# chlhnu/DOT-SOCP

Hardware: AMD Instinct MI355X
Metric: ADMM iters/sec on NxNxT dot2d staggered grid at 1/2/4/8 MI355X (higher is better)
Workload: dtype f64

## Files before the change

### dot-socp_amd/capi.py

```python
import ctypes
import os

import numpy as np

_HERE = os.path.dirname(os.path.abspath(__file__))
LIB_PATH = os.path.join(_HERE, "lib", "libdotsocp.so")

i64 = ctypes.c_longlong
dbl = ctypes.c_double
vp = ctypes.c_void_p


class DotsocpError(RuntimeError):
    def __init__(self, code, msg):
        super().__init__(f"libdotsocp error {code}: {msg}")
        self.code = code


class Problem(ctypes.Structure):
    _fields_ = [("dim", ctypes.c_int), ("weighted", ctypes.c_int),
                ("ny", i64), ("nx", i64), ("nt", i64),
                ("D", dbl), ("E", dbl), ("cScale", dbl), ("dScale", dbl),
                ("normc", dbl), ("normd", dbl)]

# ... 15 lines not shown


METHOD_INPALM, METHOD_PALM, METHOD_ACCADMM = 0, 1, 2


F_PHI, F_Q, F_ALPHA, F_Z, F_BETA, F_C, F_WEIGHT = range(7)

SYMBOLS = {
    "dotsocp_last_error": (ctypes.c_char_p, []),
    "dotsocp_version": (ctypes.c_char_p, []),
    "dotsocp_device_count": (ctypes.c_int, []),
    "dotsocp_proj_soc": (ctypes.c_int, [vp, vp, i64, i64]),
    "dotsocp_bfd": (ctypes.c_int, [vp, vp, i64, i64, i64, dbl, dbl]),
    "dotsocp_bfd_conj": (ctypes.c_int, [vp, vp, i64, i64, i64, dbl]),
    "dotsocp_bfd1d": (ctypes.c_int, [vp, vp, i64, i64, dbl, dbl]),
    "dotsocp_bfd_conj1d": (ctypes.c_int, [vp, vp, i64, i64, dbl]),
    "dotsocp_oper_poisson": (ctypes.c_int, [vp, vp, i64, i64, i64, dbl]),
    "dotsocp_dctn": (ctypes.c_int, [vp, i64, i64, i64, ctypes.c_int]),
    "dotsocp_proj_soc_dev": (ctypes.c_int, [vp, vp, i64, i64, vp]),
    "dotsocp_bfd_dev": (ctypes.c_int, [vp, vp, i64, i64, i64, dbl, dbl, vp]),
    "dotsocp_bfd_conj_dev": (ctypes.c_int, [vp, vp, i64, i64, i64, dbl, vp]),
    "dotsocp_create": (vp, [ctypes.POINTER(Problem), ctypes.c_int, ctypes.c_int]),
    "dotsocp_create_multi": (vp, [ctypes.POINTER(Problem), ctypes.c_int, ctypes.c_int]),
    "dotsocp_destroy": (None, [vp]),
    "dotsocp_rccl_unique_id": (ctypes.c_int, [vp]),
    "dotsocp_attach_rccl": (ctypes.c_int, [vp, vp, ctypes.c_int, ctypes.c_int]),
    "dotsocp_slab_range": (ctypes.c_int, [i64, ctypes.c_int, ctypes.c_int, ctypes.POINTER(i64), ctypes.POINTER(i64)]),
    "dotsocp_field_len": (i64, [ctypes.POINTER(Problem), ctypes.c_int]),
    "dotsocp_dct_algorithm": (ctypes.c_int, [i64]),
    "dotsocp_tsolve_tri_safe": (ctypes.c_int, [i64, i64, i64]),
    "dotsocp_cone_writes_beta": (ctypes.c_int, [i64, dbl, i64, ctypes.c_int, ctypes.c_int, ctypes.c_int, dbl, dbl]),
    "dotsocp_rescale_due": (ctypes.c_int, [i64, ctypes.c_int, dbl, dbl]),
    "dotsocp_qcone_form": (ctypes.c_int, [i64, dbl, i64, ctypes.c_int, ctypes.c_int, ctypes.c_int, ctypes.c_int, dbl, dbl]),
    "dotsocp_release_cache": (i64, []),
    "dotsocp_upload": (ctypes.c_int, [vp, ctypes.c_int, vp]),
    "dotsocp_upload_layers": (ctypes.c_int, [vp, ctypes.c_int, vp, i64, i64]),
    "dotsocp_download": (ctypes.c_int, [vp, ctypes.c_int, vp]),
    "dotsocp_begin": (ctypes.c_int, [vp, ctypes.POINTER(Opts)]),
    "dotsocp_begin_method": (ctypes.c_int, [vp, ctypes.POINTER(Opts), ctypes.c_int, ctypes.POINTER(AccOpts)]),
    "dotsocp_run": (ctypes.c_int, [vp, i64, ctypes.POINTER(i64)]),
    "dotsocp_recover_outputs": (ctypes.c_int, [vp, vp, vp, vp, vp, vp, vp, vp, vp]),
    "dotsocp_jump_next_level": (ctypes.c_int, [vp, vp]),
    "dotsocp_finish": (ctypes.c_int, [vp, ctypes.POINTER(Result)]),
    "dotsocp_get_history": (ctypes.c_int, [vp, vp, vp, vp, vp]),
    "dotsocp_set_profiling": (ctypes.c_int, [vp, ctypes.c_int]),
    "dotsocp_kernel_time": (ctypes.c_int, [vp, ctypes.c_char_p, ctypes.POINTER(dbl), ctypes.POINTER(i64)]),
    "dotsocp_canary_check": (ctypes.c_int, []),
    "dotsocp_poisson_phi": (ctypes.c_int, [vp]),
    "dotsocp_synchronize": (ctypes.c_int, [vp]),
}

_lib = None


def _share_torchs_hip_runtime():
    import importlib.util
    import sys
    if "torch" in sys.modules or os.environ.get("DOTSOCP_SYSTEM_HIP"):
        return
    try:
        spec = importlib.util.find_spec("torch")
    except (ImportError, ValueError):
        return
    if not spec or not spec.submodule_search_locations:
        return
    for name in ("libamdhip64.so", "libamdhip64.so.7"):
# ... 55 lines not shown
```

### dot-socp_amd/csrc/capi.hip

```cpp
#include <cstring>
#include <new>

#include "comm.h"
#include "solver.h"

using namespace dotsocp;

namespace dotsocp {
extern thread_local std::string g_last_error;
int dotsocp_slab_range_impl(i64 nt, int world, int rank, i64 *t0, i64 *t1);
}

struct dotsocp_ctx {
    Solver s;
};

static int require_device() {
    int n = 0;
    if (hipGetDeviceCount(&n) != hipSuccess || n <= 0) {
        set_error("no HIP device available (libdotsocp has no CPU fallback)");
        return DOTSOCP_ENODEVICE;
    }
    return 0;
}
// ... 234 lines not shown
    ncclUniqueId uid;
    static_assert(sizeof(uid) == 128, "ncclUniqueId is expected to be 128 bytes");
    DS_NCCL(api.GetUniqueId(&uid));
    memcpy(id, &uid, sizeof uid);
    return 0;
}

int dotsocp_attach_rccl(dotsocp_ctx *ctx, const unsigned char id[128], int rank, int world) {
    if (!ctx) { set_error("ctx is NULL"); return DOTSOCP_EINVAL; }
    return ctx->s.attach_rccl(id, rank, world);
}

#define CTX_OR_FAIL()                                      \
    do {                                                   \
        if (!ctx) { set_error("ctx is NULL"); return DOTSOCP_EINVAL; } \
        (void)hipGetLastError();    \
    } while (0)

int dotsocp_dct_algorithm(dotsocp_i64 n) { return dct_choose_algorithm(n); }
int dotsocp_tsolve_tri_safe(dotsocp_i64 ny, dotsocp_i64 nx, dotsocp_i64 nt) { return tsolve_tri_safe(ny, nx, nt) ? 1 : 0; }

int dotsocp_cone_writes_beta(dotsocp_i64 it, double last_sigma_it, dotsocp_i64 maxit, int check_step_by_step,
                             int last_of_run, int rescale, double maxFeas, double relGap) {
    return cone_writes_beta(it, last_sigma_it, maxit, check_step_by_step != 0, last_of_run != 0, rescale, maxFeas, relGap) ? 1 : 0;
}
int dotsocp_rescale_due(dotsocp_i64 it, int rescale, double maxFeas, double relGap) {
    return rescale_due(it, rescale, maxFeas, relGap) ? 1 : 0;
}
int dotsocp_qcone_form(dotsocp_i64 it, double last_sigma_it, dotsocp_i64 maxit, int check_step_by_step, int last_of_run,
                       int next_last_of_run, int rescale, double maxFeas, double relGap) {
    return qcone_form(it, last_sigma_it, maxit, check_step_by_step != 0, last_of_run != 0, next_last_of_run != 0, rescale,
                      maxFeas, relGap);
}

dotsocp_i64 dotsocp_field_len(const dotsocp_problem *p, int field) {
    if (!p || (p->dim != 1 && p->dim != 2) || p->nt < 2 || p->nx < 1 || (p->dim == 2 && p->ny < 1)) return -1;
    const i64 ny = p->dim == 1 ? p->nx : p->ny, nx = p->dim == 1 ? 1 : p->nx, nt = p->nt;
    const i64 Nphi = ny * nx * nt, Nz = ny * nx * (nt - 1);
    const i64 Nq = Nz + ny * (nx - 1) * nt + (ny - 1) * nx * nt;
    switch (field) {
        case DOTSOCP_F_PHI: case DOTSOCP_F_C: return Nphi;
        case DOTSOCP_F_Q: case DOTSOCP_F_ALPHA: case DOTSOCP_F_WEIGHT: return Nq;
        case DOTSOCP_F_Z: case DOTSOCP_F_BETA: return Nz * (p->dim == 1 ? 6 : 10);
        default: return -1;
    }
}

int dotsocp_upload(dotsocp_ctx *ctx, int field, const double *host) { CTX_OR_FAIL(); return ctx->s.upload(field, host); }
dotsocp_i64 dotsocp_release_cache(void) { return (dotsocp_i64)device_cache_release(); }

int dotsocp_upload_layers(dotsocp_ctx *ctx, int field, const double *host, dotsocp_i64 t0, dotsocp_i64 n) {
    CTX_OR_FAIL();
    return ctx->s.upload_layers(field, host, t0, n);
}
int dotsocp_download(dotsocp_ctx *ctx, int field, double *host) { CTX_OR_FAIL(); return ctx->s.download(field, host); }
int dotsocp_begin(dotsocp_ctx *ctx, const dotsocp_opts *opts) { CTX_OR_FAIL(); return ctx->s.begin(opts); }
int dotsocp_begin_method(dotsocp_ctx *ctx, const dotsocp_opts *opts, int method, const dotsocp_acc_opts *acc) {
    CTX_OR_FAIL();
    return ctx->s.begin_method(opts, method, acc);
}
int dotsocp_recover_outputs(dotsocp_ctx *ctx, const double *rho0, const double *rho1, double *rho, double *Ex,
                            double *Ey, double *q0, double *bx, double *by) {
    CTX_OR_FAIL();
    if (ctx->s.prob.dim == 1)
        return ctx->s.recover_outputs(rho0, rho1, rho, nullptr, Ex, q0, nullptr, bx);
    return ctx->s.recover_outputs(rho0, rho1, rho, Ex, Ey, q0, bx, by);
// ... 63 lines not shown
```

### dot-socp_amd/csrc/kernels.h

```cpp
#pragma once
#include "common.h"
#include "defer.h"

namespace dotsocp {

struct LoopCoef {
    double s;
    double sf;
    double dF;
    double at, ax, ay;
    double tau;
    double c1, c2;
    double dinv1, dinv2;
};

enum {
    S_Q2 = 0, S_Z2, S_APHI2, S_ALPHA2, S_BETA2, S_FBBETA2, S_PRIM1, S_PRIM2, S_DUAL1, S_DUAL2,
    S_COMPLEM, S_DOTCOMP, S_RHO2, S_RHOFQ2, S_MRHOB, S_M2, S_RHOB2, S_QALPHA, S_CPHI, S_PHI2,
    S_COUNT
};

struct KktCoef {
    double sigma;
    double kappa;
// ... 88 lines not shown
                        double sc_in1, double sc_out, hipStream_t st, i64 tc0 = 0, i64 Nzc = -1);
int launch_scale_div(double *x, const double *w, i64 n, double sc, hipStream_t st);
int launch_fill(double *x, i64 n, double v, hipStream_t st);
int launch_outputs(const Grid &g, const double *q, const double *alpha, const double *weight, const double *rho0,
                   const double *rho1, const double *a_prev, double sig, double cD, double dD, int which, double *out,
                   hipStream_t st);
int launch_out_tail(const Grid &g, const double *alpha, const double *weight, double sig, double cD, double *out,
                    hipStream_t st);

int launch_qstep_fused(const Grid &g, const LoopCoef &c, const FusedGeom &fg, const double *phi,
                       const double *q2, const double *sx, const double *sy, const double *weight,
                       const double *tail_bx, const double *tail_by, double *q_out, double *alpha,
                       hipStream_t st);
struct QStepExtra {
    ScaleOps aops;
    double *partials, *resid;
    double kappa, dsD;
    double *u0_tail;
    int c_ends;
};
int launch_qstep_rhs(const Grid &g, const LoopCoef &c, const FusedGeom &fg, const double *phi, const double *q2,
                     const double *sx, const double *sy, const double *weight, const double *tail_bx,
                     const double *tail_by, const double *cvec, double *q_out, const double *alpha_in, double *alpha_out,
                     double *rhs, hipStream_t st, i64 z0 = 0, i64 zcount = -1, i64 zstride = 1,
                     const QStepExtra *ex = nullptr);
i64 qstep_rhs_blocks(const Grid &g, const FusedGeom &fg);
struct QConeArgs {
    const double *phi, *q2v, *sx, *sy, *cvec, *alpha_in, *gamma_in;
    double *alpha_out, *rhs, *q_out, *beta_out, *q2_out, *sx_out, *sy_out;
    i64 TC;
    int ap_on;
    double ap_mul, ap_div;
    int c_ends;
};
int launch_qcone(const Grid &g, const LoopCoef &c, const FusedGeom &fg, QConeArgs a, bool gout, hipStream_t st);
i64 qcone_chunk_len(const Grid &g);
int launch_rhs_sigma_fix(const Grid &g, double *rhs, const double *r, double *cvec, double factor, hipStream_t st,
                         bool c_ends = false);
int launch_c_interior_test(const Grid &g, const double *cvec, int *flag, hipStream_t st);
i64 qstep_rhs_chunks(const Grid &g, const FusedGeom &fg, i64 *TC = nullptr);
int launch_qstep_rhs_acc(int var, const Grid &g, const LoopCoef &c, const FusedGeom &fg, const double *phi,
                         const double *q2, const double *sx, const double *sy, const double *weight, const double *cvec,
                         double *q_raw, const double *alpha_in, double *alpha_out, double *rhs, double *q_state,
                         const double *q_anchor, const double *alpha_anchor, const AccCoef &k, hipStream_t st,
                         const double *tail_bx = nullptr, const double *tail_by = nullptr, double *u0_tail = nullptr);
int launch_rhs_fixup(const Grid &g, const LoopCoef &c, const double *u0_prev, double *rhs, hipStream_t st);
int launch_qstep_palm_first(const Grid &g, const LoopCoef &c, const FusedGeom &fg, const double *phi, const double *q2,
                            const double *sx, const double *sy, const double *cvec, double *q_out, const double *alpha,
                            double *rhs, hipStream_t st, const double *tail_bx = nullptr, const double *tail_by = nullptr,
                            const double *qk = nullptr);
int launch_grad(const Grid &g, const LoopCoef &c, const double *phi, double *out, hipStream_t st);
int launch_tail_finalize(const Grid &g, const LoopCoef &c, const FusedGeom &fg, const double *q2, const double *sx,
                         const double *sy, double *tail_bx, double *tail_by, hipStream_t st);
int launch_kkt_tail(const Grid &g, const double *alpha, const double *beta, const double *weight, double *a0,
                    double *a0w, double *bt_bx, double *bt_by, hipStream_t st);
int launch_rhs(const Grid &g, const LoopCoef &c, const double *q, const double *alpha, const double *cvec,
               const double *weight, const double *u0_prev, double *rhs, hipStream_t st, bool c_ends = false);
int launch_qstep(const Grid &g, const LoopCoef &c, const double *phi, const double *z, const double *beta,
                 const double *weight, const double *tail_bx, const double *tail_by, double *q,
                 double *alpha, hipStream_t st);
int launch_u0_tail(const Grid &g, const double *q, const double *alpha, const double *weight, double *out,
                   hipStream_t st);
int launch_scale(double *x, i64 n, double mul, double div, hipStream_t st);
#define DS_MAX_WORLD 64
struct PencilCuts {
    int world;
    i64 cut[DS_MAX_WORLD + 1];
};
// ... 71 lines not shown
```

### dot-socp_amd/csrc/solver.h

```cpp
#pragma once
#include <chrono>
#include <functional>
#include <memory>
#include <string>
#include <vector>

#include "hostmem.h"
#include "kernels.h"

namespace dotsocp {

int guarded_malloc(void **p, size_t bytes);
void guarded_free(void *p);
long long device_cache_release();
int canary_check(std::string *report);
bool canary_enabled();
bool stream_stress_enabled();
void stream_stress(hipStream_t st);

template <class T>
inline int dmalloc(T **p, i64 n) {
    *p = nullptr;
    if (n <= 0) n = 1;
    return guarded_malloc((void **)p, sizeof(T) * (size_t)n);
// ... 44 lines not shown
    i64 l0 = 0, nl = 0;
    double *pencil = nullptr, *pencil2 = nullptr;
    double *stage = nullptr;
    double *u0_prev = nullptr, *tail_bx = nullptr, *tail_by = nullptr;
    double *a0_prev = nullptr, *a0w_prev = nullptr, *btail_bx = nullptr, *btail_by = nullptr;
    double *send_plane = nullptr, *send_plane2 = nullptr, *send_bx = nullptr, *send_by = nullptr;
    KktWork kw{};
    double *q_old = nullptr, *q2 = nullptr, *beta2 = nullptr, *sx = nullptr, *sy = nullptr;
    double *q3 = nullptr, *p2 = nullptr, *sxp = nullptr, *syp = nullptr;
    double *send_pbx = nullptr, *send_pby = nullptr, *ptail_bx = nullptr, *ptail_by = nullptr;
    double *alpha2 = nullptr;
    double *sx2 = nullptr, *sy2 = nullptr;
    double *tri_send = nullptr, *tri_recv = nullptr, *tri_bsend = nullptr, *tri_brecv = nullptr, *tri_zero = nullptr;
    double *carry = nullptr;
    FusedGeom fg{};
    double *phi_p = nullptr, *alpha_p = nullptr, *z_p = nullptr;
    double *phi_a = nullptr, *q_a = nullptr, *alpha_a = nullptr, *z_a = nullptr, *beta_a = nullptr;
};

#define FOR_SLABS(s) for (auto &s : slabs) if (int rc_use__ = use(s)) return rc_use__; else

int dotsocp_slab_range_impl(i64 nt, int world, int rank, i64 *t0, i64 *t1);
void pencil_range(i64 plane, int world, int j, i64 *l0, i64 *l1);

bool if_adjust_sigma(double iter, double last_iter);

enum Phase { PH_RHS = 0, PH_POISSON, PH_PROJ, PH_QSTEP, PH_BETA, PH_KKT, PH_FUSED_A, PH_FUSED_B, PH_MATERIALISE,
             PH_COMM, PH_INTERP, PH_ACC_CONE, PH_ACC_GATHER, PH_QSTEP0, PH_TRANSPOSE, PH_CONE_CARRY, PH_QCONE, PH_COUNT };

bool rescale_due(i64 it, int rescale, double maxFeas, double relGap);
bool cone_writes_beta(i64 it, double lastSigmaIt, i64 maxit, bool checkStepByStep, bool last_of_run, int rescale,
                      double maxFeas, double relGap);

enum { QCONE_NONE = 0, QCONE_STEADY = 1, QCONE_EXIT = 2 };
int qcone_form(i64 it, double lastSigmaIt, i64 maxit, bool checkStepByStep, bool last_of_run, bool next_last_of_run,
               int rescale, double maxFeas, double relGap);

struct Solver {
    dotsocp_problem prob{};
    int device = 0;
    i64 ny = 0, nx = 0, nt = 0;
    hipStream_t stream = nullptr;
    hipStream_t stream_z = nullptr;
    bool multi_device = false;
    int ndev_visible = 1;
    std::vector<DevRes *> devres;
    int cur_dev = -1;
    std::vector<Slab> slabs;
    std::unique_ptr<DeferCtx> defer;
    int world = 1;
    int rank = 0;
    void *nccl = nullptr;
    double *h_sums = nullptr;
    double *d_red = nullptr;
    bool fused = true;
    bool overlap = false;
    bool tri_tsolve = true;
    bool peer_ok = true;
    bool cross_device = false;
    ~Solver();
    int init(const dotsocp_problem *p, int device, int nslabs, bool multi_dev = false);
    int attach_rccl(const unsigned char *id, int rank, int world);
    int use(const Slab &s);
    int use_dev(int d);
    int sync_all();
    DevRes *res_for(int dev);
    i64 column_pad() const;
    i64 row_pitch() const;
    int alloc_slabs(int first, int count);
// ... 164 lines not shown
```

### dot-socp_amd/csrc/solver.hip

```cpp
#include "solver.h"

#include <algorithm>
#include <cmath>
#include <cstring>

#include "comm.h"

namespace dotsocp {

void Solver::update_coef() {
    lc.s = E / D;
    lc.sf = edge_factor(lc.s);
    lc.dF = E / dScale;
    const double ht = 1.0 / (double)(nt - 1);
    lc.at = D * (1.0 / ht);
    lc.ax = (nx > 1) ? D * (1.0 / (1.0 / (double)(nx - 1))) : 0.0;
    lc.ay = (ny > 1) ? D * (1.0 / (1.0 / (double)(ny - 1))) : 0.0;
    lc.tau = opts.tau;
    const double tmp = (E / D) * (E / D);
    if (prob.weighted) { lc.c1 = 2.0 * tmp; lc.c2 = tmp; }
    else { lc.c1 = 1.0 + 2.0 * tmp; lc.c2 = 1.0 + tmp; }
    lc.dinv1 = 1.0 / lc.c1;
    lc.dinv2 = 1.0 / lc.c2;
}
// ... 302 lines not shown
        }
        const int mode = deferred ? 1 : 0;
        if (s.carry && C > 1) {
            for (i64 z = z0; z < z0 + zc; ++z) {
                a.carry_in = (z > 0) ? s.carry : nullptr;
                a.carry_out = (z + 1 < C) ? s.carry : nullptr;
                DS_CHECK(launch_cone_fused(mode, s.g, lc, s.fg, a, s.st, z, 1, flavour));
            }
        } else {
            DS_CHECK(launch_cone_fused(mode, s.g, lc, s.fg, a, s.st, z0, zc, flavour));
        }
        if (deferred && part != 1) std::swap(s.beta, s.beta2);
    }
    prof_end(ph);
    if (part == 1) return 0;
    if (deferred) {
        bops.clear();
        beta_gamma = gout;
    }
    return 0;
}

KktCoef Solver::kkt_coef() const {
    KktCoef k;
    k.sigma = sigma;
    k.kappa = sigma * cScale * D;
    k.dsD = dScale / D;
    k.dsE = dScale / E;
    return k;
}

int Solver::phase_q(int part, bool kkt, int early) {
    if (!fused) DS_CHECK(flush_alpha());
    if (early != QCONE_NONE && (part != 0 || kkt || multi() || !fused || !deferred || !beta_gamma || !bops.empty())) {
        set_error("internal: early cone pass in a state it does not serve");
        return DOTSOCP_ESTATE;
    }
    const bool egout = (early == QCONE_STEADY);
    const int ph = (early != QCONE_NONE) ? PH_QCONE : PH_QSTEP;
    prof_begin(ph);
    FOR_SLABS(s) {
        hipStream_t st = s.st;
        if (early != QCONE_NONE && qcone != 2) {
            if (!s.sx2) {
                DS_CHECK(s.zalloc(&s.sx2, s.fg.sx_len));
                DS_CHECK(s.zalloc(&s.sy2, s.fg.sy_len));
            }
            QConeArgs a{};
            a.phi = s.phi; a.q2v = s.q2; a.sx = s.sx; a.sy = s.sy; a.cvec = s.c; a.alpha_in = s.alpha; a.gamma_in = s.beta;
            a.alpha_out = s.alpha2; a.rhs = s.w0; a.q_out = s.q_old; a.beta_out = s.beta2;
            a.q2_out = s.q; a.sx_out = s.sx2; a.sy_out = s.sy2;
            a.ap_on = aops.n; a.ap_mul = aops.mul; a.ap_div = aops.div;
            a.c_ends = (c_ends_on && s.c_ends) ? 1 : 0;
            DS_CHECK(launch_qcone(s.g, lc, s.fg, a, egout, st));
            std::swap(s.alpha, s.alpha2);
            std::swap(s.q, s.q_old);
            std::swap(s.q2, s.q_old);
            std::swap(s.sx, s.sx2);
            std::swap(s.sy, s.sy2);
            std::swap(s.beta, s.beta2);
        } else if (!fused) {
            DS_CHECK(launch_qstep(s.g, lc, s.phi, s.z, s.beta, s.weight, s.tail_bx, s.tail_by, s.q, s.alpha, s.st));
        } else {
            const i64 C = qstep_rhs_chunks(s.g, s.fg);
            i64 z0 = 0, zc = C, zs = 1;
            if (part == 1) { zc = C - 1; }
            else if (part == 2) { z0 = C - 1; zc = 1; }
            QStepExtra ex{};
            ex.aops = aops;
            ex.c_ends = (c_ends_on && s.c_ends) ? 1 : 0;
            if (multi() && !s.g.last && part != 1) ex.u0_tail = s.send_plane;
            if (kkt) {
                const KktCoef k = kkt_coef();
                ex.partials = kkt_qstep_partials(s.g, s.kw);
                ex.resid = s.w1;
                ex.kappa = k.kappa; ex.dsD = k.dsD;
            }
            DS_CHECK(launch_qstep_rhs(s.g, lc, s.fg, s.phi, s.q2, s.sx, s.sy, s.weight, s.tail_bx, s.tail_by, s.c,
                                      s.q_old, s.alpha, s.alpha2, s.w0, st, z0, zc, zs, &ex));
            if (part != 1) std::swap(s.alpha, s.alpha2);
            if (part != 1) std::swap(s.q, s.q_old);
            if (early != QCONE_NONE) {
                FusedArgs a{};
                a.q = s.q; a.q2 = s.q2; a.sx = s.sx; a.sy = s.sy;
                a.beta_in = s.beta; a.beta_out = s.beta2;
                a.bops = bops;
                DS_CHECK(launch_cone_fused(1, s.g, lc, s.fg, a, s.st, 0, s.fg.chunks, CONE_GIN | (egout ? CONE_GOUT : 0)));
                std::swap(s.beta, s.beta2);
            }
        }
    }
    prof_end(ph);
    if (part == 1) return 0;
    q_valid = true;
    if (early != QCONE_NONE) {
        q_valid = !egout || qcone == 2;
        beta_gamma = egout;
        z_valid = false;
        z_prev_ok = false;
        early_pass = true;
        early_gout = egout;
    }
    u0_made = multi() && fused;
    if (fused) aops.clear();
    rhs_valid = fused;
    if (multi() && fused && comm_z && cone_split_enabled()) halo_pending = true;
    else DS_CHECK(exchange_q_halo(true));
    return 0;
}

int Solver::phase_mult() {
    if (fused) {
        deferred = true;
        return 0;
    }
    prof_begin(PH_BETA);
    FOR_SLABS(s) DS_CHECK(launch_beta_update(s.g, lc, s.q, s.z, s.beta, s.st));
    prof_end(PH_BETA);
    return 0;
}

int Solver::materialise() {
    if (!fused || !deferred) return 0;
    DS_CHECK(need_beta_form("materialise"));
    DS_CHECK(need_q("materialise"));
    DS_CHECK(ensure_halo());
    prof_begin(PH_MATERIALISE);
    FOR_SLABS(s) {
        FusedArgs a = pending_step_args(s);
        a.beta_out = s.beta;
// ... 180 lines not shown
    dScale = dScale2 * dScale;
    cScale = cScale2 * cScale;
    sigmaScale = sigmaScale * (cScale2 / dScale2);
    update_coef();
    rescale += 1;
    return 0;
}

bool rescale_due(i64 it, int rescale, double maxFeas, double relGap) {
    if (rescale >= 3 && (it % 100) == 0) return true;
    if (rescale == 1 && maxFeas < 2e-2 && it >= 10 && relGap < 5e-2) return true;
    if (rescale == 2 && maxFeas < 5e-3 && it >= 50 && relGap < 1e-2) return true;
    return false;
}

bool cone_writes_beta(i64 it, double lastSigmaIt, i64 maxit, bool checkStepByStep, bool last_of_run, int rescale,
                      double maxFeas, double relGap) {
    if (checkStepByStep || if_adjust_sigma((double)it, lastSigmaIt) || it >= maxit) return true;
    if (last_of_run) return true;
    return rescale_due(it + 1, rescale, maxFeas, relGap);
}

int qcone_form(i64 it, double lastSigmaIt, i64 maxit, bool checkStepByStep, bool last_of_run, bool next_last_of_run,
               int rescale, double maxFeas, double relGap) {
    if (cone_writes_beta(it, lastSigmaIt, maxit, checkStepByStep, last_of_run, rescale, maxFeas, relGap)) return QCONE_NONE;
    return cone_writes_beta(it + 1, lastSigmaIt, maxit, checkStepByStep, next_last_of_run, rescale, maxFeas, relGap)
               ? QCONE_EXIT : QCONE_STEADY;
}

bool Solver::time_limit_passed() const {
    return timeout_pending || (remote() ? false : (elapsed() > time_limit || (timeout_at > 0 && it >= timeout_at)));
}

int Solver::qcone_decide() const {
    if (qcone == 0 || !fused || multi() || prob.weighted || method != DOTSOCP_METHOD_INPALM) return QCONE_NONE;
    if (!deferred || !beta_gamma || !bops.empty()) return QCONE_NONE;
    const Slab &s = slabs[0];
    if (s.g.ncl < 1 || s.fg.XB != 4) return QCONE_NONE;
    if (qcone < 0 && s.fg.nyblk * s.fg.nxblk < 2048) return QCONE_NONE;
    if (time_limit_passed()) return QCONE_NONE;
    return qcone_form(it, lastSigmaIt, opts.maxit, opts.ifCheckStepByStep != 0, last_of_run, next_last_of_run, rescale,
                      maxFeas, relGap);
}

bool if_adjust_sigma(double iter, double last_iter) {
    const double passed = iter - last_iter;
    if (iter < 20 && passed >= 3) return true;
    if (iter < 50 && passed >= 6) return true;
    if (iter < 100 && passed >= 10) return true;
    if (iter < 200 && passed >= 15) return true;
    if (iter < 500 && passed >= 25) return true;
    return passed >= 40;
}

static const double kUpdateRule[11][2] = {
    {1.1, 1.10}, {1.2, 1.15}, {1.5, 1.20}, {2, 1.26}, {2.5, 1.28}, {3.33, 1.32},
    {5, 1.35}, {10, 1.40}, {20, 1.60}, {40, 1.80}, {50, 2.00}};

static double get_factor(double xi) {
    double factor = 1.0;
    for (int i = 0; i < 11; ++i) {
        if (xi >= kUpdateRule[i][0]) factor = kUpdateRule[i][1];
        else break;
    }
    return factor;
}

static void adjust_lagrangian_param(double &sigma, double xi, double &factor) {
    factor = 1.0;
    if (xi >= 1) factor = get_factor(xi);
    else if (xi < 1) factor = 1.0 / get_factor(1.0 / xi);
    if (factor != 1.0) {
        const double old = sigma;
        sigma = std::max(std::min(sigma * factor, 1e3), 1e-3);
        factor = sigma / old;
// ... 273 lines not shown
```

### dot-socp_amd/csrc/stencil.hip

```cpp
#include "device_utils.h"
#include "gather_tile.h"
#include "kernels.h"

#include <cstdlib>

namespace dotsocp {

static inline dim3 tile_grid(const Grid &g, i64 layers) {
    return dim3((unsigned)((g.ny + TILE_Y - 1) / TILE_Y), (unsigned)((g.nx + TILE_X - 1) / TILE_X), (unsigned)layers);
}

template <bool WEIGHTED>
__global__ void __launch_bounds__(TILE_Y *TILE_X) k_rhs(RhsArgs a, double *__restrict__ rhs) {
    const i64 y = (i64)blockIdx.x * TILE_Y + threadIdx.x;
    const i64 x = (i64)blockIdx.y * TILE_X + threadIdx.y;
    const i64 tl = blockIdx.z;
    if (y >= a.g.ny || x >= a.g.nx) return;
    rhs[y + a.g.py * (x + a.g.nx * tl)] = rhs_value<WEIGHTED>(a, y, x, tl);
}

int launch_rhs(const Grid &g, const LoopCoef &c, const double *q, const double *alpha, const double *cvec,
               const double *weight, const double *u0_prev, double *rhs, hipStream_t st, bool c_ends) {
    if (g.Nphi <= 0) return 0;
    RhsArgs a{g, c.at, c.ax, c.ay, q, alpha, cvec, weight, u0_prev, c_ends ? 1 : 0};
// ... 754 lines not shown
    if (z0 < 0 || zcount <= 0 || zstride < 1 || z0 + (zcount - 1) * zstride >= chunks) return 0;
    a.TC = TC;
    a.z0 = z0;
    a.zstride = zstride;
    a.xcd = 1;
    dim3 grid((unsigned)fg.nyblk, (unsigned)fg.nxblk, (unsigned)zcount);
    dim3 blk(TILE_Y, TILE_X);
    const char *qe = getenv("DOTSOCP_QTX");
    const int qtx_env = qe ? atoi(qe) : 0;
    const int qtx = qtx_env ? qtx_env : ((fg.nyblk * fg.nxblk * zcount >= 8192 && !a.weight) ? 2 * TILE_X : TILE_X);
    if (var == 0 && !a.partials && qtx == 2 * TILE_X) {
        dim3 grid2((unsigned)fg.nyblk, (unsigned)((g.nx + 2 * TILE_X - 1) / (2 * TILE_X)), (unsigned)zcount);
        dim3 blk2(TILE_Y, 2 * TILE_X);
        if (a.weight) DS_KLAUNCH((k_qstep_rhs<true, 0, false, 2 * TILE_X>), grid2, blk2, 0, st, g, c, fg, a);
        else DS_KLAUNCH((k_qstep_rhs<false, 0, false, 2 * TILE_X>), grid2, blk2, 0, st, g, c, fg, a);
        DS_HIP(hipGetLastError());
        return 0;
    }
#define QRHS_LAUNCH(W, V) DS_KLAUNCH((k_qstep_rhs<W, V>), grid, blk, 0, st, g, c, fg, a)
    if (var == 0 && a.partials) {
        if (a.weight) DS_KLAUNCH((k_qstep_rhs<true, 0, true>), grid, blk, 0, st, g, c, fg, a);
        else DS_KLAUNCH((k_qstep_rhs<false, 0, true>), grid, blk, 0, st, g, c, fg, a);
    } else if (a.weight) {
        if (var == 0) QRHS_LAUNCH(true, 0); else if (var == 1) QRHS_LAUNCH(true, 1); else QRHS_LAUNCH(true, 2);
    } else {
        if (var == 0) QRHS_LAUNCH(false, 0); else if (var == 1) QRHS_LAUNCH(false, 1);
        else if (var == 2) QRHS_LAUNCH(false, 2); else QRHS_LAUNCH(false, 3);
    }
#undef QRHS_LAUNCH
    DS_HIP(hipGetLastError());
    return 0;
}

template <bool NT, bool GOUT>
__global__ void __launch_bounds__(TILE_Y *TILE_X, 3) k_qcone(Grid g, LoopCoef c, FusedGeom fg, QConeArgs a) {
    constexpr int XB = TILE_X;
    __shared__ double2 xch[2][XB][TILE_Y];
    __shared__ double ph[2][XB + 2][TILE_Y + 2];
    __shared__ double2 gch[2][XB][64];
    const APend ap{a.ap_on, a.ap_mul, a.ap_div};
    const int lane = threadIdx.x, xl = threadIdx.y;
    const BlockId blk = block_id(true);
    const i64 y = (i64)blk.x * TILE_Y + lane;
    const i64 x = (i64)blk.y * XB + xl;
    const bool inb = (y < g.ny) && (x < g.nx);
    const i64 t0 = (i64)blk.z * a.TC;
    const i64 t1 = (t0 + a.TC < g.ntl) ? t0 + a.TC : g.ntl;
    const i64 tstart = (t0 >= 2) ? t0 - 2 : 0;
    const i64 tstop = (t1 == g.ntl) ? t1 + 1 : t1;
    const i64 nxblk = gridDim.y, nyblk = gridDim.x;
    const bool hasBx = inb && (x < g.nx - 1), hasBy = inb && (y < g.ny - 1);
    const bool rightCol = hasBx && (xl == XB - 1), topRow = hasBy && (lane == TILE_Y - 1);
    const bool leftTile = inb && (xl == 0) && (x >= 1);
    const bool belowTile = inb && (lane == 0) && (y >= 1);
    const bool sxOwn = hasBx && ((x % fg.XB) == fg.XB - 1), syOwn = hasBy && ((y & 63) == 63);
    const i64 yc = inb ? y : 0, xc = inb ? x : 0;
    double p0 = 0.0;
    if (inb) {
        const i64 node0 = y + g.py * (x + g.nx * tstart);
        p0 = a.phi[node0];
        double hx = 0.0, hl = 0.0, hy = 0.0, hb = 0.0;
        if (rightCol) hx = a.phi[node0 + g.py];
        if (leftTile) hl = a.phi[node0 - g.py];
        if (topRow) hy = a.phi[node0 + 1];
        if (belowTile) hb = a.phi[node0 - 1];
        ph[0][xl + 1][lane + 1] = p0;
        if (xl == XB - 1) ph[0][XB + 1][lane + 1] = hx;
        if (xl == 0) ph[0][0][lane + 1] = hl;
        if (lane == TILE_Y - 1) ph[0][xl + 1][TILE_Y + 1] = hy;
        if (lane == 0) ph[0][xl + 1][0] = hb;
    }
    double u0prev = 0.0;
    double q0c = 0.0;
    EdgeQuad eprev{0.0, 0.0, 0.0, 0.0};
    GatherCarry gc;
    int par = 0;
    __syncthreads();
    for (i64 tl = tstart; tl < tstop; ++tl) {
        const bool own = tl >= t0;
        const bool hasC = (tl > tstart) && (tl - 1 < g.ncl);
        const i64 ci = yc + g.py * (xc + g.nx * (hasC ? tl - 1 : 0));
        double b[10];
        if (hasC) {
#pragma unroll
            for (int j = 0; j < 10; ++j) b[j] = ld_stream<NT>(a.gamma_in + j * g.Nc + ci);
        }
        EdgeQuad ecur{0.0, 0.0, 0.0, 0.0};
        double q0n = 0.0;
        if (tl < g.ntl) {
            const i64 node = yc + g.py * (xc + g.nx * tl);
            const bool tbnd = (g.t0 + tl == 0) || (g.t0 + tl == g.nt - 1);
            const double dc = tbnd ? c.c2 : c.c1;
            const double di = tbnd ? c.dinv2 : c.dinv1;
            const bool hasCell = inb && (tl < g.ncl);
            const i64 eX = hasBx ? g.offBx + g.bxLayer * tl + yc + g.py * xc : node;
            const i64 eY = hasBy ? g.offBy + g.byLayer * tl + yc + g.pyb * xc : node;
            const i64 k0 = hasCell ? node : 0;
            const i64 nodeT = hasCell ? node + g.plane : node;
            const double pTl = a.phi[nodeT];
            double hx = 0.0, hl = 0.0, hy = 0.0, hb = 0.0;
            if (rightCol) hx = a.phi[nodeT + g.py];
            if (leftTile) hl = a.phi[nodeT - g.py];
            if (topRow) hy = a.phi[nodeT + 1];
            if (belowTile) hb = a.phi[nodeT - 1];
            const double pXl = ph[par][xl + 2][lane + 1];
            const double pYl = ph[par][xl + 1][lane + 2];
            const double al0 = a.alpha_in[k0], alX = a.alpha_in[eX], alY = a.alpha_in[eY];
            const double g0 = a.q2v[k0];
            double gX = a.q2v[eX], gY = a.q2v[eY];
            double cv = 0.0;
            if (!a.c_ends || tbnd) cv = a.cvec[node];
            const double sxv = a.sx[sxOwn ? (tl * fg.nxblk + (x / fg.XB + 1)) * g.ny + y : 0];
            const double syv = a.sy[syOwn ? (tl * g.nx + x) * fg.nyblk + (y / 64 + 1) : 0];
            double pLl = 0.0, alL = 0.0, gL = 0.0, sxL = 0.0;
            if (leftTile) {
                const i64 eL = g.offBx + g.bxLayer * tl + y + g.py * (x - 1);
                pLl = ph[par][0][lane + 1];
                alL = a.alpha_in[eL];
                gL = a.q2v[eL];
                if (((x - 1) % fg.XB) == fg.XB - 1) sxL = a.sx[(tl * fg.nxblk + ((x - 1) / fg.XB + 1)) * g.ny + y];
            }
            double pBl = 0.0, alB = 0.0, gB = 0.0, syB = 0.0;
            if (belowTile) {
                const i64 eB = g.offBy + g.byLayer * tl + (y - 1) + g.pyb * x;
                pBl = ph[par][xl + 1][0];
                alB = a.alpha_in[eB];
                gB = a.q2v[eB];
                if (((y - 1) & 63) == 63) syB = a.sy[(tl * g.nx + x) * fg.nyblk + ((y - 1) / 64 + 1)];
            }
            if (sxOwn) gX = c.sf * (gX + sxv);
            if (syOwn) gY = c.sf * (gY + syv);
            double pT = 0.0, u0 = 0.0, ubx = 0.0, uby = 0.0;
            double a0n = 0.0, qXn = 0.0, aXn = 0.0, qYn = 0.0, aYn = 0.0;
            if (hasCell) {
                pT = pTl;
                double tmp = (-c.at) * p0;
                tmp += c.at * pT;
                q_calc<false, 0>(c, tmp, g0, c.c1, c.dinv1, 1.0, al0, ap, q0n, a0n, u0);
            }
            if (hasBx) {
                double tmp = (-c.ax) * p0;
                tmp += c.ax * pXl;
                q_calc<false, 0>(c, tmp, gX, dc, di, 1.0, alX, ap, qXn, aXn, ubx);
            }
            if (hasBy) {
                double tmp = (-c.ay) * p0;
                tmp += c.ay * pYl;
                q_calc<false, 0>(c, tmp, gY, dc, di, 1.0, alY, ap, qYn, aYn, uby);
            }
            double ubx_l = 0.0, qL = 0.0, uby_b = 0.0, qB = 0.0;
            if (leftTile) {
                double q2 = gL;
                if (((x - 1) % fg.XB) == fg.XB - 1) q2 = c.sf * (q2 + sxL);
                double tmp = (-c.ax) * pLl;
                tmp += c.ax * p0;
                double an;
                q_calc<false, 0>(c, tmp, q2, dc, di, 1.0, alL, ap, qL, an, ubx_l);
            }
            if (belowTile) {
                double q2 = gB;
                if (((y - 1) & 63) == 63) q2 = c.sf * (q2 + syB);
                double tmp = (-c.ay) * pBl;
// ... 71 lines not shown
                    for (int j = 0; j < 10; ++j) st_stream<NT>(a.beta_out + j * g.Nc + ci, b[j]);
                }
#pragma unroll
                for (int j = 0; j < 10; ++j) v[j] = v[j] - b[j];
                proj_row<10>(v);
                if (GOUT && own && inb) {
#pragma unroll
                    for (int j = 0; j < 10; ++j) st_stream<NT>(a.beta_out + j * g.Nc + ci, mult_carry(b[j], v[j], c.tau));
                }
#pragma unroll
                for (int j = 0; j < 10; ++j) w[j] = v[j] + b[j];
                if (own && inb) a.q2_out[ci] = c.s * (w[9] - w[0]);
            } else {
#pragma unroll
                for (int j = 0; j < 10; ++j) w[j] = 0.0;
            }
            gather_emit<XB>(g, c.sf, gch, gc, w, tl - 1, own && inb, x, y, xl, lane, nxblk, nyblk, blk.y, blk.x, a.q2_out,
                            a.sx_out, a.sy_out);
        }
        eprev = ecur;
        q0c = q0n;
    }
}

i64 qcone_chunk_len(const Grid &g) {
    i64 TC = g.ntl;
    if (const char *e = getenv("DOTSOCP_QCONE_TC")) {
        const i64 n = atoll(e);
        if (n >= 1) TC = n;
    }
    return TC < g.ntl ? TC : g.ntl;
}

int launch_qcone(const Grid &g, const LoopCoef &c, const FusedGeom &fg, QConeArgs a, bool gout, hipStream_t st) {
    if (fg.XB != TILE_X || !(g.first && g.last) || g.ncl < 1) { set_error("internal: k_qcone on a grid it does not serve"); return DOTSOCP_ESTATE; }
    a.TC = qcone_chunk_len(g);
    const i64 chunks = (g.ntl + a.TC - 1) / a.TC;
    dim3 grid((unsigned)fg.nyblk, (unsigned)fg.nxblk, (unsigned)chunks);
    dim3 blk(TILE_Y, TILE_X);
    const bool nt = stream_nt_enabled();
    if (gout) {
        if (nt) DS_KLAUNCH((k_qcone<true, true>), grid, blk, 0, st, g, c, fg, a);
        else DS_KLAUNCH((k_qcone<false, true>), grid, blk, 0, st, g, c, fg, a);
    } else {
        if (nt) DS_KLAUNCH((k_qcone<true, false>), grid, blk, 0, st, g, c, fg, a);
        else DS_KLAUNCH((k_qcone<false, false>), grid, blk, 0, st, g, c, fg, a);
    }
    DS_HIP(hipGetLastError());
    return 0;
}

__global__ void __launch_bounds__(TILE_Y *TILE_X) k_rhs_fixup(Grid g, double at, const double *__restrict__ u0_prev,
                                                               double *__restrict__ rhs) {
    const i64 y = (i64)blockIdx.x * TILE_Y + threadIdx.x;
    const i64 x = (i64)blockIdx.y * TILE_X + threadIdx.y;
    if (y >= g.ny || x >= g.nx) return;
    const i64 i = y + g.py * x;
    rhs[i] = rhs[i] + at * u0_prev[i];
}

int launch_rhs_fixup(const Grid &g, const LoopCoef &c, const double *u0_prev, double *rhs, hipStream_t st) {
    DS_KLAUNCH(k_rhs_fixup, tile_grid(g, 1), dim3(TILE_Y, TILE_X), 0, st, g, c.at, u0_prev, rhs);
    DS_HIP(hipGetLastError());
    return 0;
}

int launch_qstep_palm_first(const Grid &g, const LoopCoef &c, const FusedGeom &fg, const double *phi, const double *q2,
                            const double *sx, const double *sy, const double *cvec, double *q_out, const double *alpha,
                            double *rhs, hipStream_t st, const double *tail_bx, const double *tail_by, const double *qk) {
    QRhsArgs a{};
    a.phi = phi; a.q2v = q2; a.sx = sx; a.sy = sy; a.cvec = cvec; a.tail_bx = tail_bx; a.tail_by = tail_by;
    a.alpha_in = alpha; a.q_out = q_out; a.rhs = rhs; a.qk = qk;
    return launch_qstep_rhs_var(3, g, c, fg, a, st);
}

__global__ void __launch_bounds__(TILE_Y *TILE_X) k_grad(Grid g, LoopCoef c, const double *__restrict__ phi,
                                                          double *__restrict__ out) {
    const i64 y = (i64)blockIdx.x * TILE_Y + threadIdx.x;
    const i64 x = (i64)blockIdx.y * TILE_X + threadIdx.y;
// ... 132 lines not shown
```

### include/dotsocp.h

```cpp
#ifndef DOTSOCP_H
#define DOTSOCP_H

#ifdef __cplusplus
extern "C" {
#endif

typedef long long dotsocp_i64;

enum {
    DOTSOCP_OK = 0,
    DOTSOCP_EINVAL = -1,
    DOTSOCP_ENODEVICE = -2,
    DOTSOCP_EHIP = -3,
    DOTSOCP_ESTATE = -4,
    DOTSOCP_ECOMM = -5
};

const char *dotsocp_last_error(void);
const char *dotsocp_version(void);
int dotsocp_device_count(void);
dotsocp_i64 dotsocp_release_cache(void);


int dotsocp_proj_soc(double *out, const double *in, dotsocp_i64 M, dotsocp_i64 K);
// ... 65 lines not shown
};

typedef struct {
    double sigma;
    double sigma_internal;
    double cScale, dScale;
    double times[7];
    dotsocp_i64 iters;
    dotsocp_i64 hist_len;
    int stopped;
    double time_extra;
} dotsocp_result;

dotsocp_ctx *dotsocp_create(const dotsocp_problem *prob, int device, int nslabs);
dotsocp_ctx *dotsocp_create_multi(const dotsocp_problem *prob, int first_device, int ngpu);
void dotsocp_destroy(dotsocp_ctx *ctx);

int dotsocp_rccl_unique_id(unsigned char id[128]);
int dotsocp_attach_rccl(dotsocp_ctx *ctx, const unsigned char id[128], int rank, int world);

int dotsocp_slab_range(dotsocp_i64 nt, int world, int rank, dotsocp_i64 *t0, dotsocp_i64 *t1);

dotsocp_i64 dotsocp_field_len(const dotsocp_problem *prob, int field);

int dotsocp_dct_algorithm(dotsocp_i64 n);

int dotsocp_tsolve_tri_safe(dotsocp_i64 ny, dotsocp_i64 nx, dotsocp_i64 nt);

int dotsocp_cone_writes_beta(dotsocp_i64 it, double last_sigma_it, dotsocp_i64 maxit, int check_step_by_step,
                             int last_of_run, int rescale, double maxFeas, double relGap);
int dotsocp_rescale_due(dotsocp_i64 it, int rescale, double maxFeas, double relGap);
int dotsocp_qcone_form(dotsocp_i64 it, double last_sigma_it, dotsocp_i64 maxit, int check_step_by_step, int last_of_run,
                       int next_last_of_run, int rescale, double maxFeas, double relGap);

int dotsocp_upload(dotsocp_ctx *ctx, int field, const double *host);
int dotsocp_download(dotsocp_ctx *ctx, int field, double *host);
int dotsocp_upload_layers(dotsocp_ctx *ctx, int field, const double *host, dotsocp_i64 t0, dotsocp_i64 n);

int dotsocp_begin(dotsocp_ctx *ctx, const dotsocp_opts *opts);
int dotsocp_begin_method(dotsocp_ctx *ctx, const dotsocp_opts *opts, int method, const dotsocp_acc_opts *acc);
int dotsocp_run(dotsocp_ctx *ctx, dotsocp_i64 n_iters, dotsocp_i64 *done);
int dotsocp_finish(dotsocp_ctx *ctx, dotsocp_result *res);

int dotsocp_recover_outputs(dotsocp_ctx *ctx, const double *rho0, const double *rho1, double *rho, double *Ex,
                            double *Ey, double *q0, double *bx, double *by);

int dotsocp_jump_next_level(dotsocp_ctx *coarse, dotsocp_ctx *fine);

int dotsocp_get_history(dotsocp_ctx *ctx, double *kkt, double *time, double *iter, double *pdGap);

int dotsocp_set_profiling(dotsocp_ctx *ctx, int on);
int dotsocp_kernel_time(dotsocp_ctx *ctx, const char *name, double *avg_ms, dotsocp_i64 *launches);

int dotsocp_canary_check(void);

int dotsocp_poisson_phi(dotsocp_ctx *ctx);

int dotsocp_synchronize(dotsocp_ctx *ctx);

#ifdef __cplusplus
}
#endif
#endif
```

Before: 96.73.

## Add entry form of fused q-cone pass that rebuilds gamma from beta in-kernel

Adds a QCONE_ENTRY variant of the early fused q/cone kernel for iterations where the gamma carry is not yet available (beta_gamma false). In that form the kernel reads the old q and beta, applies pending scale ops, and recomputes the cone projection carry inline instead of reading gamma_in. This lets the fused early pass run on more iterations rather than falling back to the separate q-step and cone kernels. The trade-off is more arithmetic and extra q_old loads per cell, a different launch-bounds occupancy hint, and new buffer-aliasing rules. The form is on by default and can be turned off with an environment variable.

```diff
diff --git a/dot-socp_amd/capi.py b/dot-socp_amd/capi.py
--- a/dot-socp_amd/capi.py
+++ b/dot-socp_amd/capi.py
@@ -71,6 +71,7 @@
     "dotsocp_cone_writes_beta": (ctypes.c_int, [i64, dbl, i64, ctypes.c_int, ctypes.c_int, ctypes.c_int, dbl, dbl]),
     "dotsocp_rescale_due": (ctypes.c_int, [i64, ctypes.c_int, dbl, dbl]),
     "dotsocp_qcone_form": (ctypes.c_int, [i64, dbl, i64, ctypes.c_int, ctypes.c_int, ctypes.c_int, ctypes.c_int, dbl, dbl]),
+    "dotsocp_qcone_select": (ctypes.c_int, [ctypes.c_int, ctypes.c_int, ctypes.c_int]),
     "dotsocp_release_cache": (i64, []),
     "dotsocp_upload": (ctypes.c_int, [vp, ctypes.c_int, vp]),
     "dotsocp_upload_layers": (ctypes.c_int, [vp, ctypes.c_int, vp, i64, i64]),
diff --git a/dot-socp_amd/csrc/capi.hip b/dot-socp_amd/csrc/capi.hip
--- a/dot-socp_amd/csrc/capi.hip
+++ b/dot-socp_amd/csrc/capi.hip
@@ -290,6 +290,7 @@
     return qcone_form(it, last_sigma_it, maxit, check_step_by_step != 0, last_of_run != 0, next_last_of_run != 0, rescale,
                       maxFeas, relGap);
 }
+int dotsocp_qcone_select(int form, int beta_gamma, int entry_on) { return qcone_select(form, beta_gamma != 0, entry_on != 0); }
 
 dotsocp_i64 dotsocp_field_len(const dotsocp_problem *p, int field) {
     if (!p || (p->dim != 1 && p->dim != 2) || p->nt < 2 || p->nx < 1 || (p->dim == 2 && p->ny < 1)) return -1;
diff --git a/dot-socp_amd/csrc/kernels.h b/dot-socp_amd/csrc/kernels.h
--- a/dot-socp_amd/csrc/kernels.h
+++ b/dot-socp_amd/csrc/kernels.h
@@ -144,8 +144,10 @@
     int ap_on;
     double ap_mul, ap_div;
     int c_ends;
-};
-int launch_qcone(const Grid &g, const LoopCoef &c, const FusedGeom &fg, QConeArgs a, bool gout, hipStream_t st);
+    const double *q_old_in;
+    ScaleOps bops;
+};
+int launch_qcone(const Grid &g, const LoopCoef &c, const FusedGeom &fg, QConeArgs a, bool gin, bool gout, hipStream_t st);
 i64 qcone_chunk_len(const Grid &g);
 int launch_rhs_sigma_fix(const Grid &g, double *rhs, const double *r, double *cvec, double factor, hipStream_t st,
                          bool c_ends = false);
diff --git a/dot-socp_amd/csrc/solver.h b/dot-socp_amd/csrc/solver.h
--- a/dot-socp_amd/csrc/solver.h
+++ b/dot-socp_amd/csrc/solver.h
@@ -100,9 +100,10 @@
 bool cone_writes_beta(i64 it, double lastSigmaIt, i64 maxit, bool checkStepByStep, bool last_of_run, int rescale,
                       double maxFeas, double relGap);
 
-enum { QCONE_NONE = 0, QCONE_STEADY = 1, QCONE_EXIT = 2 };
+enum { QCONE_NONE = 0, QCONE_STEADY = 1, QCONE_EXIT = 2, QCONE_ENTRY = 3 };
 int qcone_form(i64 it, double lastSigmaIt, i64 maxit, bool checkStepByStep, bool last_of_run, bool next_last_of_run,
                int rescale, double maxFeas, double relGap);
+int qcone_select(int form, bool beta_gamma, bool entry_on);
 
 struct Solver {
     dotsocp_problem prob{};
diff --git a/dot-socp_amd/csrc/solver.hip b/dot-socp_amd/csrc/solver.hip
--- a/dot-socp_amd/csrc/solver.hip
+++ b/dot-socp_amd/csrc/solver.hip
@@ -358,11 +358,14 @@
 
 int Solver::phase_q(int part, bool kkt, int early) {
     if (!fused) DS_CHECK(flush_alpha());
-    if (early != QCONE_NONE && (part != 0 || kkt || multi() || !fused || !deferred || !beta_gamma || !bops.empty())) {
+    const bool entry = (early == QCONE_ENTRY);
+    if (early != QCONE_NONE && (part != 0 || kkt || multi() || !fused ||
+                                (entry ? beta_gamma : (!deferred || !beta_gamma || !bops.empty())))) {
         set_error("internal: early cone pass in a state it does not serve");
         return DOTSOCP_ESTATE;
     }
-    const bool egout = (early == QCONE_STEADY);
+    if (entry) DS_CHECK(need_q("the entry form of the early cone pass"));
+    const bool egout = (early == QCONE_STEADY || entry);
     const int ph = (early != QCONE_NONE) ? PH_QCONE : PH_QSTEP;
     prof_begin(ph);
     FOR_SLABS(s) {
@@ -378,9 +381,15 @@
             a.q2_out = s.q; a.sx_out = s.sx2; a.sy_out = s.sy2;
             a.ap_on = aops.n; a.ap_mul = aops.mul; a.ap_div = aops.div;
             a.c_ends = (c_ends_on && s.c_ends) ? 1 : 0;
-            DS_CHECK(launch_qcone(s.g, lc, s.fg, a, egout, st));
+            if (entry) {
+                a.q_old_in = s.q;
+                a.q_out = nullptr;
+                a.q2_out = s.q_old;
+                a.bops = bops;
+            }
+            DS_CHECK(launch_qcone(s.g, lc, s.fg, a, !entry, egout, st));
             std::swap(s.alpha, s.alpha2);
-            std::swap(s.q, s.q_old);
+            if (!entry) std::swap(s.q, s.q_old);
             std::swap(s.q2, s.q_old);
             std::swap(s.sx, s.sx2);
             std::swap(s.sy, s.sy2);
@@ -411,7 +420,9 @@
                 a.q = s.q; a.q2 = s.q2; a.sx = s.sx; a.sy = s.sy;
                 a.beta_in = s.beta; a.beta_out = s.beta2;
                 a.bops = bops;
-                DS_CHECK(launch_cone_fused(1, s.g, lc, s.fg, a, s.st, 0, s.fg.chunks, CONE_GIN | (egout ? CONE_GOUT : 0)));
+                if (entry) a.q_old = s.q_old;
+                DS_CHECK(launch_cone_fused(1, s.g, lc, s.fg, a, s.st, 0, s.fg.chunks,
+                                           (entry ? 0 : CONE_GIN) | (egout ? CONE_GOUT : 0)));
                 std::swap(s.beta, s.beta2);
             }
         }
@@ -422,6 +433,7 @@
     if (early != QCONE_NONE) {
         q_valid = !egout || qcone == 2;
         beta_gamma = egout;
+        bops.clear();
         z_valid = false;
         z_prev_ok = false;
         early_pass = true;
@@ -668,15 +680,24 @@
     return timeout_pending || (remote() ? false : (elapsed() > time_limit || (timeout_at > 0 && it >= timeout_at)));
 }
 
+int qcone_select(int form, bool beta_gamma, bool entry_on) {
+    if (form != QCONE_STEADY && form != QCONE_EXIT) return QCONE_NONE;
+    if (beta_gamma) return form;
+    return (entry_on && form == QCONE_STEADY) ? QCONE_ENTRY : QCONE_NONE;
+}
+
 int Solver::qcone_decide() const {
     if (qcone == 0 || !fused || multi() || prob.weighted || method != DOTSOCP_METHOD_INPALM) return QCONE_NONE;
-    if (!deferred || !beta_gamma || !bops.empty()) return QCONE_NONE;
+    if (beta_gamma ? (!deferred || !bops.empty()) : !cone_carry) return QCONE_NONE;
     const Slab &s = slabs[0];
     if (s.g.ncl < 1 || s.fg.XB != 4) return QCONE_NONE;
     if (qcone < 0 && s.fg.nyblk * s.fg.nxblk < 2048) return QCONE_NONE;
     if (time_limit_passed()) return QCONE_NONE;
-    return qcone_form(it, lastSigmaIt, opts.maxit, opts.ifCheckStepByStep != 0, last_of_run, next_last_of_run, rescale,
-                      maxFeas, relGap);
+    bool entry_on = true;
+    if (const char *e = getenv("DOTSOCP_QCONE_ENTRY")) entry_on = (atoi(e) != 0);
+    return qcone_select(qcone_form(it, lastSigmaIt, opts.maxit, opts.ifCheckStepByStep != 0, last_of_run, next_last_of_run,
+                                   rescale, maxFeas, relGap),
+                        beta_gamma, entry_on);
 }
 
 bool if_adjust_sigma(double iter, double last_iter) {
diff --git a/dot-socp_amd/csrc/stencil.hip b/dot-socp_amd/csrc/stencil.hip
--- a/dot-socp_amd/csrc/stencil.hip
+++ b/dot-socp_amd/csrc/stencil.hip
@@ -810,8 +810,9 @@
     return 0;
 }
 
-template <bool NT, bool GOUT>
-__global__ void __launch_bounds__(TILE_Y *TILE_X, 3) k_qcone(Grid g, LoopCoef c, FusedGeom fg, QConeArgs a) {
+template <bool NT, bool GIN, bool GOUT>
+__global__ void __launch_bounds__(TILE_Y *TILE_X, GIN ? 3 : 2) k_qcone(Grid g, LoopCoef c, FusedGeom fg, QConeArgs a) {
+    static_assert(GIN || GOUT, "the early pass behind a beta-writing pass exists in the gamma-writing form only");
     constexpr int XB = TILE_X;
     __shared__ double2 xch[2][XB][TILE_Y];
     __shared__ double ph[2][XB + 2][TILE_Y + 2];
@@ -851,6 +852,8 @@
     double u0prev = 0.0;
     double q0c = 0.0;
     EdgeQuad eprev{0.0, 0.0, 0.0, 0.0};
+    EdgeQuad curo{0.0, 0.0, 0.0, 0.0};
+    if constexpr (!GIN) curo = load_edges(g, a.q_old_in, yc, xc, tstart, c.sf);
     GatherCarry gc;
     int par = 0;
     __syncthreads();
@@ -862,6 +865,12 @@
         if (hasC) {
 #pragma unroll
             for (int j = 0; j < 10; ++j) b[j] = ld_stream<NT>(a.gamma_in + j * g.Nc + ci);
+        }
+        double q0o = 0.0;
+        EdgeQuad nxto{0.0, 0.0, 0.0, 0.0};
+        if constexpr (!GIN) {
+            q0o = a.q_old_in[ci];
+            nxto = load_edges(g, a.q_old_in, yc, xc, hasC ? tl : tstart, c.sf);
         }
         EdgeQuad ecur{0.0, 0.0, 0.0, 0.0};
         double q0n = 0.0;
@@ -906,6 +915,19 @@
                 gB = a.q2v[eB];
                 if (((y - 1) & 63) == 63) syB = a.sy[(tl * g.nx + x) * fg.nyblk + ((y - 1) / 64 + 1)];
             }
+            if constexpr (!GIN) {
+                if (hasC) {
+                    apply_scale_ops(b, a.bops);
+                    double zo[10];
+                    build_z2(zo, q0o, curo, nxto, c.s, c.dF);
+#pragma unroll
+                    for (int j = 0; j < 10; ++j) zo[j] = zo[j] - b[j];
+                    proj_row<10>(zo);
+#pragma unroll
+                    for (int j = 0; j < 10; ++j) b[j] = mult_carry(b[j], zo[j], c.tau);
+                    curo = nxto;
+                }
+            }
             if (sxOwn) gX = c.sf * (gX + sxv);
             if (syOwn) gY = c.sf * (gY + syv);
             double pT = 0.0, u0 = 0.0, ubx = 0.0, uby = 0.0;
@@ -1043,19 +1065,27 @@
     return TC < g.ntl ? TC : g.ntl;
 }
 
-int launch_qcone(const Grid &g, const LoopCoef &c, const FusedGeom &fg, QConeArgs a, bool gout, hipStream_t st) {
+int launch_qcone(const Grid &g, const LoopCoef &c, const FusedGeom &fg, QConeArgs a, bool gin, bool gout, hipStream_t st) {
     if (fg.XB != TILE_X || !(g.first && g.last) || g.ncl < 1) { set_error("internal: k_qcone on a grid it does not serve"); return DOTSOCP_ESTATE; }
+    if (!gin && (!gout || !a.q_old_in || a.beta_out == a.gamma_in || a.q2_out == a.q_old_in)) {
+        set_error("internal: the entry form of k_qcone with the buffers of another form");
+        return DOTSOCP_ESTATE;
+    }
+    if (gin) a.bops.clear();
     a.TC = qcone_chunk_len(g);
     const i64 chunks = (g.ntl + a.TC - 1) / a.TC;
     dim3 grid((unsigned)fg.nyblk, (unsigned)fg.nxblk, (unsigned)chunks);
     dim3 blk(TILE_Y, TILE_X);
     const bool nt = stream_nt_enabled();
-    if (gout) {
-        if (nt) DS_KLAUNCH((k_qcone<true, true>), grid, blk, 0, st, g, c, fg, a);
-        else DS_KLAUNCH((k_qcone<false, true>), grid, blk, 0, st, g, c, fg, a);
+    if (!gin) {
+        if (nt) DS_KLAUNCH((k_qcone<true, false, true>), grid, blk, 0, st, g, c, fg, a);
+        else DS_KLAUNCH((k_qcone<false, false, true>), grid, blk, 0, st, g, c, fg, a);
+    } else if (gout) {
+        if (nt) DS_KLAUNCH((k_qcone<true, true, true>), grid, blk, 0, st, g, c, fg, a);
+        else DS_KLAUNCH((k_qcone<false, true, true>), grid, blk, 0, st, g, c, fg, a);
     } else {
-        if (nt) DS_KLAUNCH((k_qcone<true, false>), grid, blk, 0, st, g, c, fg, a);
-        else DS_KLAUNCH((k_qcone<false, false>), grid, blk, 0, st, g, c, fg, a);
+        if (nt) DS_KLAUNCH((k_qcone<true, true, false>), grid, blk, 0, st, g, c, fg, a);
+        else DS_KLAUNCH((k_qcone<false, true, false>), grid, blk, 0, st, g, c, fg, a);
     }
     DS_HIP(hipGetLastError());
     return 0;
diff --git a/include/dotsocp.h b/include/dotsocp.h
--- a/include/dotsocp.h
+++ b/include/dotsocp.h
@@ -121,6 +121,7 @@
 int dotsocp_rescale_due(dotsocp_i64 it, int rescale, double maxFeas, double relGap);
 int dotsocp_qcone_form(dotsocp_i64 it, double last_sigma_it, dotsocp_i64 maxit, int check_step_by_step, int last_of_run,
                        int next_last_of_run, int rescale, double maxFeas, double relGap);
+int dotsocp_qcone_select(int form, int beta_gamma, int entry_on);
 
 int dotsocp_upload(dotsocp_ctx *ctx, int field, const double *host);
 int dotsocp_download(dotsocp_ctx *ctx, int field, double *host);
```

Result: no change. 97.65 (median of 6 runs) (+0.9%).
